# eradiate/eradiate-kernel

Measured on AMD Instinct MI355X. Metric: Msamples/s volpath 512x512x1024spp plane-parallel atmosphere, higher is better.
Workload: dtype f32; 1 GPU; C3 volpath heterogeneous 128^3 grid + HG g=0.8, 512x512x1024spp; integrator=volpath, sampler=independent seed 0, block_size=32, rfilter=box

## Files before the change

eradiate-kernel_amd/csrc/pmath.h:

```cpp
#pragma once
#include <stdint.h>
#include <math.h>
#include <string.h>

#if defined(__HIPCC__)
#  define PM_HD __host__ __device__ inline
#else
#  define PM_HD static inline
#endif

PM_HD uint32_t pm_bits(float x) { return __builtin_bit_cast(uint32_t, x); }
PM_HD float pm_from_bits(uint32_t u) { return __builtin_bit_cast(float, u); }
PM_HD uint64_t pm_bits_d(double x) { return __builtin_bit_cast(uint64_t, x); }
PM_HD double pm_from_bits_d(uint64_t u) { return __builtin_bit_cast(double, u); }

PM_HD float pm_fma(float a, float b, float c) { return __builtin_fmaf(a, b, c); }
PM_HD float pm_sqrt(float x) { return __builtin_sqrtf(x); }
PM_HD float pm_rcp(float x) {
#if defined(__HIP_DEVICE_COMPILE__) && !defined(PM_RCP_BY_DIVISION)
    const float y0 = __builtin_amdgcn_rcpf(x);
    const float e = __builtin_fmaf(-x, y0, 1.0f);
    return __builtin_amdgcn_div_fixupf(__builtin_fmaf(e, y0, y0), x, 1.0f);
#else
    return 1.0f / x;
#endif
}
PM_HD float pm_rsqrt(float x) { return pm_rcp(__builtin_sqrtf(x)); }
PM_HD float pm_abs(float x) { return pm_from_bits(pm_bits(x) & 0x7fffffffu); }

PM_HD float pm_invariant_rcp(float d) {
    const uint32_t b = pm_bits(d), e = (b >> 23) & 0xffu;
    const float rd = 1.0f / d;
    const uint32_t er = (pm_bits(rd) >> 23) & 0xffu;
    return (d > 0.f && e >= 67u && e <= 187u && er >= 67u && er <= 187u && (b & 0x7fffffu) != 0x7fffffu) ? rd : 0.f;
}
PM_HD float pm_div_by_invariant(float x, float d, float rd) {
    if (rd == 0.f || pm_bits(x) * 2u - 0x41000000u >= 0x7c000000u) return x / d;
    float q = x * rd;
    float r = pm_fma(-q, d, x);
    q = pm_fma(r, rd, q);
    r = pm_fma(-q, d, x);
    q = pm_fma(r, rd, q);
    return q;
}
PM_HD float pm_min(float a, float b) { return b < a ? b : a; }
PM_HD float pm_max(float a, float b) { return a < b ? b : a; }
PM_HD float pm_safe_sqrt(float x) { return __builtin_sqrtf(pm_max(x, 0.0f)); }
PM_HD float pm_floor(float x) { return __builtin_floorf(x); }
PM_HD float pm_ceil(float x) { return __builtin_ceilf(x); }
PM_HD float pm_inf() { return pm_from_bits(0x7f800000u); }
PM_HD float pm_nan() { return pm_from_bits(0x7fc00000u); }
PM_HD int pm_isfinite(float x) { return (pm_bits(x) & 0x7f800000u) != 0x7f800000u; }

PM_HD float pm_sign(float x) { return pm_from_bits((pm_bits(x) & 0x80000000u) | 0x3f800000u); }
PM_HD float pm_mulsign(float a, float b) { return pm_from_bits(pm_bits(a) ^ (pm_bits(b) & 0x80000000u)); }
PM_HD float pm_mulsign_neg(float a, float b) { return pm_from_bits(pm_bits(a) ^ (~pm_bits(b) & 0x80000000u)); }

PM_HD double pm_fma_d(double a, double b, double c) { return __builtin_fma(a, b, c); }

PM_HD double pm_log_core_cr(uint32_t ix) {
    int e = (int) (ix >> 23) - 126;
    float mf = pm_from_bits((ix & 0x007fffffu) | 0x3f000000u);
    if (mf < 0.707106781186547524f) { e -= 1; mf = mf + mf; }
    float tf = mf + 1.0f;
    float yf = pm_fma(pm_fma(0x1.deab9f5bac12fp-4f, tf, -0x1.71e431e019c40p-1f), tf, 0x1.7a4e362d364a6p+0f);
    yf = pm_fma(yf, pm_fma(-tf, yf, 1.0f), yf);
    double m = (double) mf, t = m + 1.0, y = (double) yf;
    y = pm_fma_d(y, pm_fma_d(-t, y, 1.0), y);
    y = pm_fma_d(y, pm_fma_d(-t, y, 1.0), y);
    double s = (m - 1.0) * y;
    double z = s * s;
    double p = 0x1.58dd5ccd0ae5bp-3;
    p = pm_fma_d(p, z, 0x1.7322766efc727p-3);
    p = pm_fma_d(p, z, 0x1.c722d2919c869p-3);
    p = pm_fma_d(p, z, 0x1.249240ad6fd9fp-2);
    p = pm_fma_d(p, z, 0x1.999999a448740p-2);
    p = pm_fma_d(p, z, 0x1.5555555552cebp-1);
    p = pm_fma_d(p, z, 0x1.0000000000001p+1);
    return pm_fma_d((double) e, 0.69314718055994530942, s * p);
}

PM_HD float pm_log_cr(float x) {
    uint32_t ix = pm_bits(x);
    if (ix >= 0x7f800000u) {
        if (ix == 0x7f800000u) return x;
        if ((ix << 1) == 0u) return -pm_inf();
        return pm_nan();
    }
    if (ix < 0x00800000u) return -pm_inf();
    return (float) pm_log_core_cr(ix);
}

PM_HD double pm_exp_d_cr(double x) {
    double fn = __builtin_floor(pm_fma_d(x, 1.44269504088896340736, 0.5));
    double r = pm_fma_d(fn, -0.693147180369123816490, x);
    r = pm_fma_d(fn, -1.90821492927058770002e-10, r);
    double p = 0x1.2727a88044faap-22;
    p = pm_fma_d(p, r, 0x1.72f98543deccbp-19);
    p = pm_fma_d(p, r, 0x1.a01b6ce393267p-16);
    p = pm_fma_d(p, r, 0x1.a0197a4e9bd9dp-13);
    p = pm_fma_d(p, r, 0x1.6c16c0c0acbd4p-10);
    p = pm_fma_d(p, r, 0x1.1111112d4977ep-7);
    p = pm_fma_d(p, r, 0x1.55555555933c2p-5);
    p = pm_fma_d(p, r, 0x1.555555554bc09p-3);
    p = pm_fma_d(p, r, 0x1.ffffffffffe17p-2);
    p = pm_fma_d(p, r, 0x1.000000000001dp+0);
    p = pm_fma_d(p, r, 1.0);
    int64_t n = (int64_t) (int) fn;
    return pm_from_bits_d(pm_bits_d(p) + ((uint64_t) n << 52));
}

PM_HD float pm_exp_cr(float x) {
    if (!(x == x)) return x;
    if (x > 88.7228317f) return pm_inf();
    if (x < -87.3365402f) return 0.0f;
    double r = pm_exp_d_cr((double) x);
    return r < 1.17549435082228750797e-38 ? 0.0f : (float) r;
}

PM_HD void pm_sincos_cr(float x, float *s_out, float *c_out) {
    double xd = (double) x;
    double fj = __builtin_floor(pm_fma_d(xd, 0.63661977236758134308, 0.5));
    double r = pm_fma_d(fj, -1.57079632673412561417, xd);
    r = pm_fma_d(fj, -6.07710050650619224932e-11, r);
    double z = r * r;
    double sp = -0x1.a950a7cb0bcc1p-26;
// ... 30 lines not shown
    float af = pm_from_bits(ax);
    float rf = pm_from_bits(0x54a232a0u - ax / 3u);
    for (int i = 0; i < 2; ++i) {
        float ar3 = af * rf * rf * rf;
        rf = rf * pm_fma(ar3, -0.333333333f, 1.33333333f);
    }
    double a = (double) af, r = (double) rf;
    for (int i = 0; i < 2; ++i) {
        double ar3 = a * r * r * r;
        r = r * pm_fma_d(ar3, -0.33333333333333333333, 1.33333333333333333333);
    }
    float y = (float) (a * r * r);
    return pm_from_bits(pm_bits(y) | sign);
}

PM_HD float pm_pow_cr(float x, float y) {
    if ((pm_bits(y) & 0x7fffffffu) < 0x00800000u) return 1.0f;
    if (!(x == x) || !(y == y)) return pm_nan();
    if (pm_bits(x) > 0x807fffffu) return pm_nan();
    if (pm_bits(x) < 0x00800000u)
        return y > 0.0f ? 0.0f : pm_inf();
    if (pm_bits(x) == 0x7f800000u) return y > 0.0f ? pm_inf() : 0.0f;
    double t = (double) y * pm_log_core_cr(pm_bits(x));
    if (t > 88.8) return pm_inf();
    if (t < -87.3365402) return 0.0f;
    float r = (float) pm_exp_d_cr(t);
    return r < 1.17549435e-38f ? 0.0f : r;
}

#define PM_LOGF_TAB_INIT {  \
    0x1.661ec79f8f3bep+0, -0x1.57bf7808caadep-2, 0x1.571ed4aaf883dp+0, -0x1.2bef0a7c06ddbp-2, \
    0x1.49539f0f010bp+0, -0x1.01eae7f513a67p-2, 0x1.3c995b0b80385p+0, -0x1.b31d8a68224e9p-3, \
    0x1.30d190c8864a5p+0, -0x1.6574f0ac07758p-3, 0x1.25e227b0b8eap+0, -0x1.1aa2bc79c81p-3, \
    0x1.1bb4a4a1a343fp+0, -0x1.a4e76ce8c0e5ep-4, 0x1.12358f08ae5bap+0, -0x1.1973c5a611cccp-4, \
    0x1.0953f419900a7p+0, -0x1.252f438e10c1ep-5, 0x1p+0, 0x0p+0, \
    0x1.e608cfd9a47acp-1, 0x1.aa5aa5df25984p-5, 0x1.ca4b31f026aap-1, 0x1.c5e53aa362eb4p-4, \
    0x1.b2036576afce6p-1, 0x1.526e57720db08p-3, 0x1.9c2d163a1aa2dp-1, 0x1.bc2860d22477p-3, \
    0x1.886e6037841edp-1, 0x1.1058bc8a07ee1p-2, 0x1.767dcf5534862p-1, 0x1.4043057b6ee09p-2 }
#define PM_LOG2F_TAB_INIT {  \
    -0x1.efec65b963019p-2, -0x1.b0b6832d4fca4p-2, -0x1.7418b0a1fb77bp-2, -0x1.39de91a6dcf7bp-2, \
    -0x1.01d9bf3f2b631p-2, -0x1.97c1d1b3b7afp-3, -0x1.2f9e393af3c9fp-3, -0x1.960cbbf788d5cp-4, \
    -0x1.a6f9db6475fcep-5, 0x0p+0, 0x1.338ca9f24f53dp-4, 0x1.476a9543891bap-3, \
    0x1.e840b4ac4e4d2p-3, 0x1.40645f0c6651cp-2, 0x1.88e9c2c1b9ff8p-2, 0x1.ce0a44eb17bccp-2 }
#define PM_EXP2F_TAB_INIT {  \
    0x3ff0000000000000ull, 0x3fefd9b0d3158574ull, 0x3fefb5586cf9890full, 0x3fef9301d0125b51ull, \
    0x3fef72b83c7d517bull, 0x3fef54873168b9aaull, 0x3fef387a6e756238ull, 0x3fef1e9df51fdee1ull, \
    0x3fef06fe0a31b715ull, 0x3feef1a7373aa9cbull, 0x3feedea64c123422ull, 0x3feece086061892dull, \
    0x3feebfdad5362a27ull, 0x3feeb42b569d4f82ull, 0x3feeab07dd485429ull, 0x3feea47eb03a5585ull, \
    0x3feea09e667f3bcdull, 0x3fee9f75e8ec5f74ull, 0x3feea11473eb0187ull, 0x3feea589994cce13ull, \
    0x3feeace5422aa0dbull, 0x3feeb737b0cdc5e5ull, 0x3feec49182a3f090ull, 0x3feed503b23e255dull, \
    0x3feee89f995ad3adull, 0x3feeff76f2fb5e47ull, 0x3fef199bdd85529cull, 0x3fef3720dcef9069ull, \
    0x3fef5818dcfba487ull, 0x3fef7c97337b9b5full, 0x3fefa4afa2a490daull, 0x3fefd0765b6e4540ull }
static const double pm_host_logf_tab[32] = PM_LOGF_TAB_INIT;
static const double pm_host_log2f_tab[16] = PM_LOG2F_TAB_INIT;
static const uint64_t pm_host_exp2f_tab[32] = PM_EXP2F_TAB_INIT;
#if defined(__HIPCC__)
static __constant__ const double pm_dev_logf_tab[32] = PM_LOGF_TAB_INIT;
static __constant__ const double pm_dev_log2f_tab[16] = PM_LOG2F_TAB_INIT;
static __constant__ const uint64_t pm_dev_exp2f_tab[32] = PM_EXP2F_TAB_INIT;
#endif
#if defined(__HIP_DEVICE_COMPILE__) && defined(PM_TABLES_IN_LDS)
__shared__ __attribute__((aligned(16))) double pm_lds_logf_tab[32];
__shared__ __attribute__((aligned(16))) uint64_t pm_lds_exp2f_tab[32];
__device__ inline void pm_tables_to_lds(uint32_t tid) {
    if (tid < 32u) { pm_lds_logf_tab[tid] = pm_dev_logf_tab[tid]; pm_lds_exp2f_tab[tid] = pm_dev_exp2f_tab[tid]; }
}
#  define PM_LOGF_TAB pm_lds_logf_tab
#  define PM_LOG2F_TAB pm_dev_log2f_tab
#  define PM_EXP2F_TAB pm_lds_exp2f_tab
#elif defined(__HIP_DEVICE_COMPILE__)
__device__ inline void pm_tables_to_lds(uint32_t) {}
#  define PM_LOGF_TAB pm_dev_logf_tab
#  define PM_LOG2F_TAB pm_dev_log2f_tab
#  define PM_EXP2F_TAB pm_dev_exp2f_tab
#else
#  if defined(__HIPCC__)
__device__ inline void pm_tables_to_lds(uint32_t) {}
#  endif
#  define PM_LOGF_TAB pm_host_logf_tab
#  define PM_LOG2F_TAB pm_host_log2f_tab
#  define PM_EXP2F_TAB pm_host_exp2f_tab
#endif

PM_HD float pm_log(float x) {
#if defined(PM_USE_LIBM) && !defined(__HIPCC__)
    return logf(x);
#endif
#if defined(PM_CORRECTLY_ROUNDED)
    return pm_log_cr(x);
#endif
    uint32_t ix = pm_bits(x);
    if (__builtin_expect(ix - 0x00800000u >= 0x7f000000u, 0)) {
        if (ix == 0x7f800000u) return x;
        if ((ix << 1) == 0u) return -pm_inf();
        if (ix < 0x00800000u) return -pm_inf();
        return pm_nan();
    }
    uint32_t tmp = ix - 0x3f330000u;
    uint32_t i = (tmp >> 19) & 15u;
    int k = (int32_t) tmp >> 23;
    double z = (double) pm_from_bits(ix - (tmp & 0xff800000u));
    double invc = PM_LOGF_TAB[2 * i], logc = PM_LOGF_TAB[2 * i + 1];
    double r = pm_fma_d(z, invc, -1.0);
    double y0 = pm_fma_d((double) k, 0x1.62e42fefa39efp-1, logc);
    double r2 = r * r;
    double y = pm_fma_d(0x1.5575b0be00b6ap-2, r, -0x1.ffffef20a4123p-2);
    y = pm_fma_d(-0x1.00ea348b88334p-2, r2, y);
    y = pm_fma_d(y, r2, y0 + r);
    return (float) y;
}

PM_HD double pm_exp2_tail(uint64_t ki, double r, double c0, double c1, double c2) {
    double s = pm_from_bits_d(PM_EXP2F_TAB[ki & 31u] + (ki << 47));
    double z = pm_fma_d(c0, r, c1);
    double r2 = r * r;
    double y = pm_fma_d(c2, r, 1.0);
    y = pm_fma_d(z, r2, y);
    return y * s;
}

PM_HD float pm_exp(float x) {
#if defined(PM_USE_LIBM) && !defined(__HIPCC__)
    return expf(x);
#endif
#if defined(PM_CORRECTLY_ROUNDED)
    return pm_exp_cr(x);
#endif
    if (__builtin_expect((pm_bits(x) & 0x7fffffffu) > 0x42aeac4fu, 0)) {
        if (!(x == x)) return x;
        if (x > 88.7228317f) return pm_inf();
        if (x < 0.0f) return 0.0f;
    }
    double xd = (double) x;
    double z = 0x1.71547652b82fep+5 * xd;
    double kd = z + 0x1.8p+52;
    uint64_t ki = pm_bits_d(kd);
    kd = kd - 0x1.8p+52;
    double r = pm_fma_d(0x1.71547652b82fep+5, xd, -kd);
    double y = pm_exp2_tail(ki, r, 0x1.c6af84b912394p-20, 0x1.ebfce50fac4f3p-13, 0x1.62e42ff0c52d6p-6);
    return y < 1.17549435082228750797e-38 ? 0.0f : (float) y;
}

PM_HD float pm_sinf_poly(double x, double x2, bool neg, int n) {
    if ((n & 1) == 0) {
        double x3 = x * x2;
        double s1 = pm_fma_d(x2, -0x1.994eb3774cf24p-13, 0x1.1107605230bc4p-7);
        double x7 = x3 * x2;
        double s = pm_fma_d(x3, -0x1.555545995a603p-3, x);
        return (float) pm_fma_d(x7, s1, s);
    }
    double sg = neg ? -1.0 : 1.0;
    double x4 = x2 * x2;
    double c2 = pm_fma_d(x2, sg * 0x1.99343027bf8c3p-16, sg * -0x1.6c087e89a359dp-10);
    double c1 = pm_fma_d(x2, sg * -0x1.ffffffd0c621cp-2, sg);
    double x6 = x4 * x2;
    double c = pm_fma_d(x4, sg * 0x1.55553e1068f19p-5, c1);
    return (float) pm_fma_d(x6, c2, c);
}

PM_HD void pm_sincos(float x, float *s_out, float *c_out) {
#if defined(PM_USE_LIBM) && !defined(__HIPCC__)
    *s_out = sinf(x); *c_out = cosf(x); return;
#endif
#if defined(PM_CORRECTLY_ROUNDED)
    pm_sincos_cr(x, s_out, c_out); return;
#endif
    uint32_t top = (pm_bits(x) >> 20) & 0x7ffu;
    double xd = (double) x;
    if (top < 0x3f4u) {
        if (top < 0x398u) { *s_out = x; *c_out = 1.0f; return; }
        double x2 = xd * xd;
        *s_out = pm_sinf_poly(xd, x2, false, 0);
        *c_out = pm_sinf_poly(xd, x2, false, 1);
        return;
    }
    if (top >= 0x42fu) { pm_sincos_cr(x, s_out, c_out); return; }
    double r = xd * 0x1.45f306dc9c883p+23;
    int n = ((int32_t) r + 0x800000) >> 24;
    xd = pm_fma_d(-(double) n, 0x1.921fb54442d18p+0, xd);
    double sg = ((n + 1) & 2) ? -1.0 : 1.0;
    double x2 = xd * xd;
    *s_out = pm_sinf_poly(xd * sg, x2, (n & 2) != 0, n);
    *c_out = pm_sinf_poly(xd * sg, x2, (n & 2) != 0, n ^ 1);
}

PM_HD float pm_cbrt(float x) {
#if defined(PM_USE_LIBM) && !defined(__HIPCC__)
    return cbrtf(x);
#endif
#if defined(PM_CORRECTLY_ROUNDED)
    return pm_cbrt_cr(x);
#endif
    uint32_t ix = pm_bits(x);
    uint32_t sign = ix & 0x80000000u;
    uint32_t ax = ix & 0x7fffffffu;
    if (ax >= 0x7f800000u) return x;
    if (ax < 0x00800000u) return pm_from_bits(sign);
    int xe = (int) (ax >> 23) - 126;
    float xm = pm_from_bits((ax & 0x007fffffu) | 0x3f000000u);
    float u = (float) (0.492659620528969547 + (0.697570460207922770 - 0.191502161678719066 * (double) xm) * (double) xm);
    float t2 = u * u * u;
    int rem = xe % 3, q = xe / 3;
    double f = rem == 0 ? 1.0 : rem == 1 ? 1.2599210498948731648 : rem == 2 ? 1.5874010519681994748
             : rem == -1 ? 1.0 / 1.2599210498948731648 : 1.0 / 1.5874010519681994748;
    float ym = (float) ((double) u * ((double) t2 + 2.0 * (double) xm) / (2.0 * (double) t2 + (double) xm) * f);
    float y = ym * pm_from_bits((uint32_t) (q + 127) << 23);
    return pm_from_bits(pm_bits(y) | sign);
}

PM_HD float pm_pow(float x, float y) {
#if defined(PM_USE_LIBM) && !defined(__HIPCC__)
    return powf(x, y);
#endif
#if defined(PM_CORRECTLY_ROUNDED)
    return pm_pow_cr(x, y);
#endif
    if ((pm_bits(y) & 0x7fffffffu) < 0x00800000u) return 1.0f;
    if (!(x == x) || !(y == y)) return pm_nan();
    if (pm_bits(x) > 0x807fffffu) return pm_nan();
    uint32_t ix = pm_bits(x);
    if (ix < 0x00800000u)
        return y > 0.0f ? 0.0f : pm_inf();
    if (ix == 0x7f800000u) return y > 0.0f ? pm_inf() : 0.0f;
// ... 25 lines not shown
```

eradiate-kernel_amd/csrc/volpath_flat.h:

```cpp
#pragma once
#include "integrator_dev.h"

namespace mtsamd {
inline namespace MTS_VARIANT_NS {

#if MTS_SPEC_N == 3
#define MTS_CX
#define MTS_CXI(id)
#define MTS_SPEC_DW 3
#else
#define MTS_CX , cx
#define MTS_CXI(id) , cx, (id)
#define MTS_SPEC_DW 4
#endif

#if MTS_SPEC_N == 3
#define MTS_FILM_STRIDE(sc) ((size_t) 5)
#else
#define MTS_FILM_STRIDE(sc) ((size_t) (sc).film_channels)
#endif
#ifndef MTS_CHAIN
#define MTS_CHAIN 1
#endif
#ifndef MTS_REPEAT_MIN_W
#define MTS_REPEAT_MIN_W 32
#endif
#define MTS_REPEAT_MIN 32

enum : uint32_t { S_TOP = 0, S_MED = 1, S_SURF = 2, S_PHASE = 3, S_BSDF = 4, S_DIRB = 5, S_NEW = 6, S_DONE = 7, S_SCATTER = 8,
                  S_ENDNEE = 9, S_ENDDIR0 = 10 };
enum : uint32_t { M_MAIN = 0, M_NEE = 1, M_DIR = 2 };
enum : uint32_t { FL_ALIVE = 1, FL_VALID_RAY = 2, FL_SPEC_CHAIN = 4, FL_NEEDS_INT = 8, FL_FROM_MEDIUM = 16 };

struct MedStep { float t, mint; F3 p; Spec sigma_t, sigma_s, combined; uint32_t info; float inv_combined ; };

DEV float div_by_invariant(float x, float d, float rd) { return pm_div_by_invariant(x, d, rd); }
DEV Spec div_by_invariant(Spec x, Spec d, float rd) {
    if (rd == 0.f) return x / d;
#if MTS_SPEC_N == 3
    return f3(div_by_invariant(x.x, d.x, rd), div_by_invariant(x.y, d.x, rd), div_by_invariant(x.z, d.x, rd));
#else
    return spec4(div_by_invariant(x.x, d.x, rd), div_by_invariant(x.y, d.x, rd), div_by_invariant(x.z, d.x, rd), div_by_invariant(x.w, d.x, rd));
#endif
}
enum : uint32_t { MI_HOMOGENEOUS = 1, MI_SPECTRAL = 2, MI_SAMPLE_EMITTERS = 4, MI_GREY = 8, MI_PHASE_SHIFT = 8 + 8 };

#if defined(MTSAMD_BLOCKSTATS)
__device__ unsigned long long g_blockstats[48];
#endif

struct GridCell { int32_t r00, r10, r01, r11, x0, x1; F3 w0, w1; };
DEV GridCell grid_cell_clamp(const float *w2l, int affine, int nx, int ny, int nz, int sx , F3 p_world) {
    F3 p = affine ? mat_point_affine(w2l, p_world) : mat_point(w2l, p_world);
    p = f3(pm_fma(p.x, (float) nx, -.5f), pm_fma(p.y, (float) ny, -.5f), pm_fma(p.z, (float) nz, -.5f));
    int ix = (int) pm_floor(p.x), iy = (int) pm_floor(p.y), iz = (int) pm_floor(p.z);
    GridCell c;
    c.w1 = p - f3((float) ix, (float) iy, (float) iz); c.w0 = f3(1.f - c.w1.x, 1.f - c.w1.y, 1.f - c.w1.z);
    c.x0 = min(max(ix, 0), nx - 1); c.x1 = min(max(ix + 1, 0), nx - 1);
    int y0 = min(max(iy, 0), ny - 1), y1 = min(max(iy + 1, 0), ny - 1), z0 = min(max(iz, 0), nz - 1), z1 = min(max(iz + 1, 0), nz - 1);
    c.r00 = (z0 * ny + y0) * sx; c.r10 = (z0 * ny + y1) * sx; c.r01 = (z1 * ny + y0) * sx; c.r11 = (z1 * ny + y1) * sx;
    return c;
}
DEV GridCell grid_cell(const DVolume &v, F3 p_world) {
    F3 p = v.affine ? mat_point_affine(v.w2l, p_world) : mat_point(v.w2l, p_world);
    const int nx = v.nx, ny = v.ny, nz = v.nz;
    p = f3(pm_fma(p.x, (float) nx, -.5f), pm_fma(p.y, (float) ny, -.5f), pm_fma(p.z, (float) nz, -.5f));
    int ix = (int) pm_floor(p.x), iy = (int) pm_floor(p.y), iz = (int) pm_floor(p.z);
    GridCell c;
    c.w1 = p - f3((float) ix, (float) iy, (float) iz); c.w0 = f3(1.f - c.w1.x, 1.f - c.w1.y, 1.f - c.w1.z);
    c.x0 = wrap_coord(v.wrap, ix, nx); c.x1 = wrap_coord(v.wrap, ix + 1, nx);
    int y0 = wrap_coord(v.wrap, iy, ny), y1 = wrap_coord(v.wrap, iy + 1, ny), z0 = wrap_coord(v.wrap, iz, nz), z1 = wrap_coord(v.wrap, iz + 1, nz);
    c.r00 = (z0 * ny + y0) * nx; c.r10 = (z0 * ny + y1) * nx; c.r01 = (z1 * ny + y0) * nx; c.r11 = (z1 * ny + y1) * nx;
    return c;
}
DEV float grid_fetch1(const MTS_GLOBAL_AS float *__restrict__ D, const GridCell &c) {
    return trilerp(D[c.r00 + c.x0], D[c.r00 + c.x1], D[c.r10 + c.x0], D[c.r10 + c.x1],
                   D[c.r01 + c.x0], D[c.r01 + c.x1], D[c.r11 + c.x0], D[c.r11 + c.x1], c.w0, c.w1);
}

typedef float mts_float4 __attribute__((ext_vector_type(4)));
typedef mts_float4 __attribute__((aligned(8))) mts_float4_a8;
DEV void grid_fetch_pair(const MTS_GLOBAL_AS float *__restrict__ P, const GridCell &c, int nx, bool columns_equal, float &sigma_t, float &albedo) {
    const int xb = min(c.x0, nx - 2);
    const bool hi0 = c.x0 != xb, hi1 = c.x1 != xb;
    mts_float4 q00 = *(const MTS_GLOBAL_AS mts_float4_a8 *) (P + 2 * (c.r00 + xb)), q01 = *(const MTS_GLOBAL_AS mts_float4_a8 *) (P + 2 * (c.r01 + xb)), q10 = q00, q11 = q01;
    if (!columns_equal) { q10 = *(const MTS_GLOBAL_AS mts_float4_a8 *) (P + 2 * (c.r10 + xb)); q11 = *(const MTS_GLOBAL_AS mts_float4_a8 *) (P + 2 * (c.r11 + xb)); }
    sigma_t = trilerp(hi0 ? q00.z : q00.x, hi1 ? q00.z : q00.x, hi0 ? q10.z : q10.x, hi1 ? q10.z : q10.x,
                      hi0 ? q01.z : q01.x, hi1 ? q01.z : q01.x, hi0 ? q11.z : q11.x, hi1 ? q11.z : q11.x, c.w0, c.w1);
    albedo = trilerp(hi0 ? q00.w : q00.y, hi1 ? q00.w : q00.y, hi0 ? q10.w : q10.y, hi1 ? q10.w : q10.y,
                     hi0 ? q01.w : q01.y, hi1 ? q01.w : q01.y, hi0 ? q11.w : q11.y, hi1 ? q11.w : q11.y, c.w0, c.w1);
}

template <bool COUNT>
DEV MedStep medium_step(const DScene &sc, const DMedium m, const DRay &ray, float sample, uint32_t channel, bool want_albedo, Counters &cnt,
                        const SpecCtx &cx = SpecCtx()) {
    MedStep mi;
#if (MTS_TRAITS & MT_MEDIA) && MTS_SPEC_N == 3
    const bool m_homogeneous = false, m_pair = true, m_grey = true, m_spectral = true;
#elif MTS_TRAITS & MT_MEDIA
    const bool m_homogeneous = false, m_pair = false, m_grey = false, m_spectral = true;
#elif MTS_TRAITS & MT_HOMOG
    const bool m_homogeneous = true, m_pair = false, m_grey = m.grey != 0, m_spectral = m.has_spectral_extinction != 0;
#else
    const bool m_homogeneous = m.is_homogeneous != 0, m_pair = m.pair_grid != nullptr, m_grey = m.grey != 0, m_spectral = m.has_spectral_extinction != 0;
#endif
    bool active = true; float mint = 0.f, maxt = pm_inf();
    if (!m_homogeneous) {
        active = bbox_ray_intersect(m.aabb, ray, mint, maxt);
        active = active && (pm_isfinite(mint) || pm_isfinite(maxt));
        if (!active) { mint = 0.f; maxt = pm_inf(); }
    }
    mint = pm_max(ray.mint, mint);
    maxt = pm_min(ray.maxt, maxt);
    Spec combined = m_homogeneous ? volume_eval(cload(sc.volumes + m.sigma_t), ray.o MTS_CXI(m.sigma_t)) * m.scale : spec_s(m.max_density);
    float mext = pick(combined, channel);
// ... 431 lines not shown
        if (MODEK == 1 && p.mode == M_MAIN) return;
        const uint32_t max_depth = (uint32_t) sc.integrator.max_depth;
        const float u = p.rng.next_1d();
        MedStep mi;
        const SpecCtx cx = ctx(p); (void) cx;
        WATERFALL_BEGIN(p.medium, mu)
            mi = medium_step<COUNT>(sc, cload(sc.media + mu), p.ray, u, p.channel, MODEK == 0 ? true : (MODEK == 1 ? false : p.mode == M_MAIN), cnt MTS_CX);
        WATERFALL_END
        if (p.si.t < mi.t) mi.t = pm_inf();
        const MediumKind mk = { mi.info };
        const bool spectral = mk.spectral(), homogeneous = mk.homogeneous(), grey = mk.grey();
        const Spec sigma_n = homogeneous ? spec_s(0.f) : mi.combined - mi.sigma_t;
        const uint32_t channel = p.channel;
        const bool is_main = MODEK == 0 ? true : (MODEK == 1 ? false : p.mode == M_MAIN), is_nee = MODEK == 0 ? false : p.mode == M_NEE;
        const float remaining_dist = is_nee ? p.ray.maxt : pm_inf();
        Spec weight = is_main ? p.thr : p.trans;
        if (spectral) {
            float t = pm_min(mi.t, p.si.t);
            if (is_nee) t = pm_min(remaining_dist, t);
            t = t - mi.mint;
            const bool surface_first = p.si.t < mi.t || mi.t > remaining_dist;
            if (grey || !homogeneous) {
                float tr = pm_exp(-t * mi.combined.x);
                float tr_pdf = surface_first ? tr : tr * mi.combined.x;
                weight = weight * (tr_pdf > 0.f ? tr * pm_rcp(tr_pdf) : 0.f);
            } else {
                Spec tr = transmittance_exp(t, mi.combined);
                Spec free_flight_pdf = surface_first ? tr : tr * mi.combined;
                float tr_pdf = pick(free_flight_pdf, channel);
                weight = weight * (tr_pdf > 0.f ? tr / tr_pdf : spec_s(0.f));
            }
        }
        float u2 = 0.f;
        if (is_main) u2 = p.rng.next_1d();
        if (is_nee) {
            if (mi.t > remaining_dist && mi.t != pm_inf()) p.wa = p.wb;
            if (mi.t > remaining_dist) mi.t = pm_inf();
        }
        const bool valid = mi.t != pm_inf();
        if (!valid) {
            if (is_main) p.thr = weight; else p.trans = weight;
            p.st = S_SURF;
            return;
        }
        const bool real_scatter = is_main && !(u2 >= (grey ? div_by_invariant(mi.sigma_t.x, mi.combined.x, mi.inv_combined)
                                                                : div_by_invariant(pick(mi.sigma_t, channel), pick(mi.combined, channel), mi.inv_combined)));
        if (!real_scatter) {
            if (grey) {
                if (is_main) { if (spectral) weight = weight * ((sigma_n.x * mi.combined.x) * pm_rcp(sigma_n.x)); }
                else { if (spectral) weight = weight * sigma_n.x; else weight = weight * div_by_invariant(sigma_n.x, mi.combined.x, mi.inv_combined); }
            } else {
                if (is_main) { if (spectral) weight = weight * (sigma_n * pick(mi.combined, channel) / pick(sigma_n, channel)); }
                else { if (spectral) weight = weight * sigma_n; else weight = weight * div_by_invariant(sigma_n, mi.combined, mi.inv_combined); }
            }
            if (is_nee) p.wa += mi.t;
            p.ray.o = mi.p; p.ray.mint = 0.f; p.si.t = p.si.t - mi.t;
            p.st = S_TOP;
            if (is_main) p.thr = weight;
            else {
                p.trans = weight;
                if (!any_nonzero(weight)) {
                    if (DEFER) p.st = is_nee ? S_ENDNEE : S_ENDDIR0;
                    else if (is_nee) end_nee(p, e); else end_direct(p, e, spec_s(0.f), 0.f);
                }
            }
            return;
        }
        p.depth += 1;
        if (!(p.depth < max_depth)) { p.thr = weight; p.flags &= ~FL_ALIVE; p.st = S_TOP; return; }
        if (grey) {
            if (spectral) weight = weight * ((mi.sigma_s.x * mi.combined.x) * pm_rcp(mi.sigma_t.x));
            else weight = weight * (mi.sigma_s.x / mi.sigma_t.x);
        } else {
            if (spectral) weight = weight * (mi.sigma_s * pick(mi.combined, channel) / pick(mi.sigma_t, channel));
            else weight = weight * (mi.sigma_s / mi.sigma_t);
        }
        p.thr = weight;
        const bool sample_emitters = (mi.info & MI_SAMPLE_EMITTERS) != 0;
        p.flags |= FL_VALID_RAY;
        p.flags = sample_emitters ? (p.flags & ~FL_SPEC_CHAIN) : (p.flags | FL_SPEC_CHAIN);
        p.ray.o = mi.p;
        p.st = sample_emitters ? S_SCATTER : S_PHASE;
    }
    template <class E> DEV void blk_scatter(PathState &p, const E &e) const {
        if (p.st != S_SCATTER) return;
        p.st = S_PHASE;
        Spec emitter_val;
        const SpecCtx cx = ctx(p); (void) cx;
        DirSample ds = sample_emitter_direction(sc, p.ray.o, p.rng.next_2d(), false, emitter_val MTS_CX);
        if (ds.pdf == 0.f) return;
        float phase_val = 0.f;
        WATERFALL_BEGIN(p.medium, mu)
            phase_val = phase_eval<true>(sc, cload(sc.media + mu).phase, -p.ray.d, p.ray.o, ds.d MTS_CX);
        WATERFALL_END
        e.cold.put_spec(C_CW, p.thr * phase_val); e.cold.put_spec(C_EMIT, emitter_val);
        e.cold.put3(C_SO, p.ray.o); e.cold.put3(C_SD, p.ray.d); e.cold.f(C_SMED) = __int_as_float(p.medium);
        p.trans = spec_s(1.f); p.wa = 0.f; p.wb = ds.dist;
        p.ray = spawn_ray(p.ray.o, ds.d); p.ray.mint = 0.f;
        queue_intersection(p);
        p.flags |= FL_FROM_MEDIUM;
        p.mode = M_NEE; p.st = S_TOP;
    }
    template <class E> DEV void blk_wsurf(PathState &p, const E &e) const {
        if (p.st != S_SURF || p.mode == M_MAIN || (p.flags & FL_NEEDS_INT)) return;
        const bool hit = hit_valid(p.si);
        const bool is_nee = p.mode == M_NEE;
        if (is_nee) p.wa += p.si.t;
        int emitter = is_nee ? -1 : sc.environment;
        Surf sf; sf.wi = -p.ray.d; sf.sh.n = f3s(0.f); sf.n = f3s(0.f);
        Spec nt = spec_s(0.f); int is_tr = 0, ext = -1, inte = -1;
        if (hit) {
            WATERFALL_BEGIN(p.si.shape, su)
                const DShape s = cload(sc.shapes + su);
                if (!is_nee) emitter = s.emitter;
                nt = s.bsdf_type == MTS_BSDF_NULL ? spec_s(1.f) : spec_s(0.f);
                is_tr = s.is_medium_transition; ext = s.exterior; inte = s.interior;
                if (emitter >= 0) complete_surface(sc, s, p.si, p.ray.d, sf);
                else if (is_tr) sf.n = hit_geo_normal(sc, s, p.si);
            WATERFALL_END
        }
        if (emitter >= 0) {
            const F3 ref_p = e.cold.get3(C_SO);
            DirSample ds;
            ds.p = p.si.p; ds.n = sf.sh.n; ds.d = p.si.p - ref_p; ds.dist = norm(ds.d); ds.d = ds.d / ds.dist;
            if (!hit) ds.d = -sf.wi;
            ds.emitter = emitter; ds.pdf = 0.f; ds.delta = false;
            const SpecCtx cx = ctx(p); (void) cx;
            end_direct(p, e, emitter_eval(sc, emitter, sf.wi.z MTS_CX), pdf_emitter_direction(sc, ref_p, ds));
            return;
        }
        if (hit) {
            p.trans = p.trans * nt;
            p.ray = spawn_ray(p.si.p, p.ray.d);
            queue_intersection(p);
            if (is_tr) p.medium = dot(p.ray.d, sf.n) > 0 ? ext : inte;
        }
        if (hit && any_nonzero(p.trans)) p.st = S_TOP;
        else if (is_nee) end_nee(p, e);
        else end_direct(p, e, spec_s(0.f), 0.f);
    }
    template <class E> DEV void blk_surf(PathState &p, const E &e) const {
        if (p.st != S_SURF || p.mode != M_MAIN || (p.flags & FL_NEEDS_INT)) return;
        const uint32_t max_depth = (uint32_t) sc.integrator.max_depth;
        const bool hit = hit_valid(p.si);
        Surf sf; sf.wi = -p.ray.d; sf.n = f3s(0.f); sf.sh.s = sf.sh.t = sf.sh.n = f3s(0.f);
        int emitter = sc.environment, bsdf_id = 0;
        if (hit) {
            WATERFALL_BEGIN(p.si.shape, su)
                const DShape s = cload(sc.shapes + su);
                emitter = s.emitter; bsdf_id = s.bsdf;
                if (s.emitter >= 0 || (s.bsdf_flags & F_Smooth) != 0) complete_surface(sc, s, p.si, p.ray.d, sf);
            WATERFALL_END
        }
        const SpecCtx cx = ctx(p); (void) cx;
        if ((p.flags & FL_SPEC_CHAIN) && emitter >= 0) p.res = p.res + p.thr * emitter_eval(sc, emitter, sf.wi.z MTS_CX);
        if (!hit) { p.flags &= ~FL_ALIVE; p.st = S_TOP; return; }
        p.st = S_BSDF;
        bool active_e = false;
        WATERFALL_BEGIN(bsdf_id, bu)
            active_e = (cload(sc.bsdfs + bu).flags & F_Smooth) != 0 && (p.depth + 1 < max_depth);
        WATERFALL_END
        if (!active_e) return;
        Spec emitter_val;
        DirSample ds = sample_emitter_direction(sc, p.si.p, p.rng.next_2d(), false, emitter_val MTS_CX);
        if (ds.pdf == 0.f) return;
        F3 wo = to_local(sf.sh, ds.d);
// ... 239 lines not shown
        if (M & G_MAXT) p.ray.maxt = f(H_MAXT);
        if (M & G_SIT) p.si.t = f(H_SIT);
        if (M & G_SIX) { p.si.p = get3(H_SIX); p.si.uv.x = f(H_SIX + 3); p.si.uv.y = f(H_SIX + 4); p.si.shape = (int) u(H_SIX + 5); p.si.prim = (int) u(H_SIX + 6); }
        if (M & G_MED) p.medium = (int) u(H_MEDIUM);
        if (M & G_THR) p.thr = get_spec(H_THR);
        if (M & G_RES) p.res = get_spec(H_RES);
        if (M & G_ETA) p.eta = f(H_ETA);
        if (M & G_TRANS) p.trans = get_spec(H_TRANS);
        if (M & G_WA) p.wa = f(H_WA);
        if (M & G_WB) p.wb = f(H_WB);
#if MTS_SPEC_N != 3
        if (M & G_WL) p.wl = get_spec(H_WL);
#endif
    }
    DEV void store(const PathState &p, int cls) const { store_m<G_ALL>(p, cls); }
    DEV void load(PathState &p) const { load_m<G_ALL>(p); }
};

struct WgArgs {
    DScene sc; const DBlock *blocks; uint32_t n_blocks, block_size, sample_count; float *film; float *cold_g; uint32_t cold_stride;
    unsigned long long *counters;
    const uint32_t *stop_flag;
    const uint32_t *tiles; uint32_t n_tiles;
};
#define MTS_TILE_PIXELS 16u

template <int WG>
DEV bool wg_env(const WgArgs &a, uint32_t wg_base, uint32_t pid, PathEnvT<ColdStoreHbm> &e) {
    const uint32_t ppb = a.block_size * a.block_size;
    e.sample_count = a.sample_count; e.film = as_global(a.film);
    e.cold.base = as_global(a.cold_g) + (size_t) (wg_base + pid) * MTS_COLD_RECORD; e.cold.stride = 1;
    __builtin_assume(((uintptr_t) e.cold.base & 127u) == 0);
    e.park = as_global(a.cold_g) + ((size_t) a.cold_stride + wg_base + pid) * MTS_COLD_RECORD;
    e.lx = e.ly = 0; e.index = 0;
    if (a.tiles != nullptr) {
        const uint32_t slot = (wg_base + pid) / MTS_TILE_PIXELS;
        if (slot >= a.n_tiles) return false;
        const uint32_t ent = as_global(a.tiles)[slot];
        if (ent == 0xFFFFFFFFu) return false;
        const MTS_GLOBAL_AS int32_t *bp = (const MTS_GLOBAL_AS int32_t *) as_global(a.blocks + (ent >> 12));
        e.blk.ox = bp[0]; e.blk.oy = bp[1]; e.blk.sx = bp[2]; e.blk.sy = bp[3]; e.blk.id = (uint32_t) bp[4]; e.blk.sample_base = (uint32_t) bp[5];
        e.blk.film_off_lo = (uint32_t) bp[6]; e.blk.film_off_hi = (uint32_t) bp[7];
        e.index = ((ent & 4095u) * MTS_TILE_PIXELS) | (pid & (MTS_TILE_PIXELS - 1u));
    } else {
        const uint32_t b = wg_base >> (uint32_t) __builtin_ctz(ppb);
        e.index = (wg_base & (ppb - 1u)) + pid;
        if (b >= a.n_blocks) return false;
        e.blk = cload(a.blocks + b);
    }
    e.film += ((size_t) e.blk.film_off_hi << 32) | e.blk.film_off_lo;
    e.lx = compact_bits(e.index); e.ly = compact_bits(e.index >> 1);
    return e.lx < (uint32_t) e.blk.sx && e.ly < (uint32_t) e.blk.sy;
}

DEV const MTS_CONST_AS void *block_uniforms(const MTS_CONST_AS void *kernarg_, uint32_t wg_base_, uint32_t &wg_base) {
    const uint64_t ka = (uint64_t) (uintptr_t) kernarg_;
    uint32_t ka_lo = (uint32_t) __builtin_amdgcn_readfirstlane((int) (uint32_t) ka), ka_hi = (uint32_t) __builtin_amdgcn_readfirstlane((int) (uint32_t) (ka >> 32));
    asm volatile("" : "+s"(ka_lo), "+s"(ka_hi));
    const MTS_CONST_AS void *kernarg = (const MTS_CONST_AS void *) (uintptr_t) ((uint64_t) ka_lo | ((uint64_t) ka_hi << 32));
    wg_base = (uint32_t) __builtin_amdgcn_readfirstlane((int) wg_base_);
    return kernarg;
}

template <bool COUNT, int WG, int C, bool WF = false, bool MOMENT = false>
#ifndef WG_BLOCK_ATTR
#define WG_BLOCK_ATTR __forceinline__
#endif
static __device__ WG_BLOCK_ATTR int wg_block(const MTS_CONST_AS void *kernarg_, uint32_t *hot_lds, uint32_t wg_base_, uint32_t pid, Counters *cnt) {
    uint32_t wg_base;
    const MTS_CONST_AS void *kernarg = block_uniforms(kernarg_, wg_base_, wg_base);
    const WgArgs a = cload_k<WgArgs>(kernarg);
    VolpathMachine<COUNT, MOMENT> vm(a.sc, *cnt);
    PathEnvT<ColdStoreHbm> e; wg_env<WG>(a, wg_base, pid, e);
    HotStore<WG> hs; hs.base = hot_lds + pid;
    typedef ClassFields<C> CF;
    PathState p;
    if (COUNT && C == B_MED) MTS_SEG_BEGIN(*cnt);
    hs.template load_m<CF::load>(p);
    if (WF && C != B_INT) p.rng.inc = wavefront_increment(a.sc.sensor, e.blk, e.lx, e.ly, __float_as_uint(e.cold.f(C_SAMPLE)));
    if (COUNT && C == B_MED) MTS_SEG(*cnt, 0);
    int cls;
#pragma nounroll
    for (int rounds = 0;; ++rounds) {
        vm.template run<CF::defer, true>(p, e, C);
        if (COUNT && C == B_MED) MTS_SEG(*cnt, 3);
        vm.template top<CF::defer>(p, e);
        if (MTS_FUSE_INT && (C == B_PHASE || C == B_SCATTER || C == B_WSURF || C == B_SURF || C == B_NEW) && a.sc.bvh_node_count == 0) {
            vm.blk_int(p, e);
            vm.template top<CF::defer>(p, e);
        }
        if (COUNT && C == B_MED) MTS_SEG(*cnt, 4);
        cls = vm.classify(p);
        if ((MTS_CHAIN & 16) && C == B_SURF) {
            if (cls != C || rounds >= 1) break;
            continue;
        }
        if ((MTS_CHAIN & 1) && C == B_WSURF) {
            if (cls != C || rounds >= 1) break;
            continue;
        }
        if (!(C == B_MED || C == B_MEDW) || cls != C || rounds >= 16) break;
        if (__popcll(__ballot(true)) < (C == B_MEDW ? MTS_REPEAT_MIN_W : MTS_REPEAT_MIN)) break;
    }
    bool chained = false;
    if ((MTS_CHAIN & 4) && C == B_MEDW && cls == B_WSURF) {
        hs.template load_add<G_ALL & ~CF::load>(p);
#pragma nounroll
        for (int r = 0; r < 2; ++r) {
            vm.blk_wsurf(p, e);
            vm.top(p, e);
            cls = vm.classify(p);
            if (cls != B_WSURF) break;
        }
        chained = true;
    }
    if ((MTS_CHAIN & 2) && (C == B_WSURF || chained) && cls == B_PHASE) {
        vm.blk_phase(p, e);
        vm.top(p, e);
        cls = vm.classify(p);
    }
    if ((MTS_CHAIN & 8) && C == B_MED && cls == B_SCATTER) {
        vm.blk_scatter(p, e);
        vm.template top<true>(p, e);
        cls = vm.classify(p);
        hs.template store_m<CF::store | ClassFields<B_SCATTER>::store>(p, cls);
    } else
    if (chained) hs.template store_m<G_ALL>(p, cls);
    else hs.template store_m<CF::store>(p, cls);
    if (COUNT && C == B_MED) MTS_SEG(*cnt, 5);
    if (CF::defer && (p.st == S_ENDNEE || p.st == S_ENDDIR0)) {
        PathState q;
        hs.template load_m<G_ALL>(q);
        if (WF) q.rng.inc = wavefront_increment(a.sc.sensor, e.blk, e.lx, e.ly, __float_as_uint(e.cold.f(C_SAMPLE)));
        vm.finish(q, e);
        vm.top(q, e);
        cls = vm.classify(q);
        hs.template store_m<G_ALL>(q, cls);
    }
    return cls;
}

template <bool COUNT_, int WG_, bool WF, bool MOMENT = false>
struct VolpathRing {
    static constexpr bool COUNT = COUNT_;
    static constexpr int WG = WG_, HOT_DWORDS = H_COUNT, PACKED = H_PACKED;
    typedef PathState State;
    typedef HotStore<WG_> Hot;
    typedef VolpathMachine<COUNT_, MOMENT> Machine;
    template <int NT> DEV static void check_shape() { static_assert(NT <= WG_, "a thread per path at most"); }
    DEV static void init_idle(State &p) {
        p.medium = -1; p.thr = p.res = p.trans = spec_s(0.f); p.eta = 1.f; p.depth = 0; p.channel = 0; p.mode = M_MAIN; p.flags = 0; p.wa = p.wb = 0.f;
#if MTS_SPEC_N != 3
        p.wl = spec_s(0.f);
#endif
    }
    template <int C> static constexpr auto block = &wg_block<COUNT_, WG_, C, WF, MOMENT>;
};

}
}
```

Measured before the change: 639.9 Msamples/s.

## Add branchless fast path for medium delta-tracking steps with rare-case fallback

Adds a specialised step_fast routine for the B_MED and B_MEDW classes in RGB media builds. It fuses medium sampling, grid lookup, transmittance, Russian roulette and state transitions into one straight-line, select-based sequence. The log, exp and invariant-division helpers gain flag variants, so the special-case checks become a single rare flag. Lanes that hit edge cases fall back to the original blk_med and top path under a wave-wide ballot. This aims to cut divergence and state-machine overhead in the hot medium loop, at the cost of duplicated logic that must stay numerically equivalent to the general path.

```diff
diff --git a/eradiate-kernel_amd/csrc/pmath.h b/eradiate-kernel_amd/csrc/pmath.h
--- a/eradiate-kernel_amd/csrc/pmath.h
+++ b/eradiate-kernel_amd/csrc/pmath.h
@@ -34,14 +34,21 @@
     const uint32_t er = (pm_bits(rd) >> 23) & 0xffu;
     return (d > 0.f && e >= 67u && e <= 187u && er >= 67u && er <= 187u && (b & 0x7fffffu) != 0x7fffffu) ? rd : 0.f;
 }
-PM_HD float pm_div_by_invariant(float x, float d, float rd) {
-    if (rd == 0.f || pm_bits(x) * 2u - 0x41000000u >= 0x7c000000u) return x / d;
+PM_HD float pm_div_by_invariant_core(float x, float d, float rd) {
     float q = x * rd;
     float r = pm_fma(-q, d, x);
     q = pm_fma(r, rd, q);
     r = pm_fma(-q, d, x);
     q = pm_fma(r, rd, q);
     return q;
+}
+PM_HD float pm_div_by_invariant(float x, float d, float rd) {
+    if (rd == 0.f || pm_bits(x) * 2u - 0x41000000u >= 0x7c000000u) return x / d;
+    return pm_div_by_invariant_core(x, d, rd);
+}
+PM_HD float pm_div_by_invariant_flag(float x, float d, float rd, bool *ok) {
+    *ok = !(pm_bits(x) * 2u - 0x41000000u >= 0x7c000000u);
+    return pm_div_by_invariant_core(x, d, rd);
 }
 PM_HD float pm_min(float a, float b) { return b < a ? b : a; }
 PM_HD float pm_max(float a, float b) { return a < b ? b : a; }
@@ -238,20 +245,7 @@
 #  define PM_EXP2F_TAB pm_host_exp2f_tab
 #endif
 
-PM_HD float pm_log(float x) {
-#if defined(PM_USE_LIBM) && !defined(__HIPCC__)
-    return logf(x);
-#endif
-#if defined(PM_CORRECTLY_ROUNDED)
-    return pm_log_cr(x);
-#endif
-    uint32_t ix = pm_bits(x);
-    if (__builtin_expect(ix - 0x00800000u >= 0x7f000000u, 0)) {
-        if (ix == 0x7f800000u) return x;
-        if ((ix << 1) == 0u) return -pm_inf();
-        if (ix < 0x00800000u) return -pm_inf();
-        return pm_nan();
-    }
+PM_HD float pm_log_core(uint32_t ix) {
     uint32_t tmp = ix - 0x3f330000u;
     uint32_t i = (tmp >> 19) & 15u;
     int k = (int32_t) tmp >> 23;
@@ -265,6 +259,31 @@
     y = pm_fma_d(y, r2, y0 + r);
     return (float) y;
 }
+PM_HD float pm_log(float x) {
+#if defined(PM_USE_LIBM) && !defined(__HIPCC__)
+    return logf(x);
+#endif
+#if defined(PM_CORRECTLY_ROUNDED)
+    return pm_log_cr(x);
+#endif
+    uint32_t ix = pm_bits(x);
+    if (__builtin_expect(ix - 0x00800000u >= 0x7f000000u, 0)) {
+        if (ix == 0x7f800000u) return x;
+        if ((ix << 1) == 0u) return -pm_inf();
+        if (ix < 0x00800000u) return -pm_inf();
+        return pm_nan();
+    }
+    return pm_log_core(ix);
+}
+PM_HD float pm_log_flag(float x, bool *ok) {
+#if (defined(PM_USE_LIBM) && !defined(__HIPCC__)) || defined(PM_CORRECTLY_ROUNDED)
+    *ok = true; return pm_log(x);
+#else
+    const uint32_t ix = pm_bits(x);
+    *ok = !(ix - 0x00800000u >= 0x7f000000u);
+    return pm_log_core(ix);
+#endif
+}
 
 PM_HD double pm_exp2_tail(uint64_t ki, double r, double c0, double c1, double c2) {
     double s = pm_from_bits_d(PM_EXP2F_TAB[ki & 31u] + (ki << 47));
@@ -275,18 +294,7 @@
     return y * s;
 }
 
-PM_HD float pm_exp(float x) {
-#if defined(PM_USE_LIBM) && !defined(__HIPCC__)
-    return expf(x);
-#endif
-#if defined(PM_CORRECTLY_ROUNDED)
-    return pm_exp_cr(x);
-#endif
-    if (__builtin_expect((pm_bits(x) & 0x7fffffffu) > 0x42aeac4fu, 0)) {
-        if (!(x == x)) return x;
-        if (x > 88.7228317f) return pm_inf();
-        if (x < 0.0f) return 0.0f;
-    }
+PM_HD float pm_exp_core(float x) {
     double xd = (double) x;
     double z = 0x1.71547652b82fep+5 * xd;
     double kd = z + 0x1.8p+52;
@@ -295,6 +303,28 @@
     double r = pm_fma_d(0x1.71547652b82fep+5, xd, -kd);
     double y = pm_exp2_tail(ki, r, 0x1.c6af84b912394p-20, 0x1.ebfce50fac4f3p-13, 0x1.62e42ff0c52d6p-6);
     return y < 1.17549435082228750797e-38 ? 0.0f : (float) y;
+}
+PM_HD float pm_exp(float x) {
+#if defined(PM_USE_LIBM) && !defined(__HIPCC__)
+    return expf(x);
+#endif
+#if defined(PM_CORRECTLY_ROUNDED)
+    return pm_exp_cr(x);
+#endif
+    if (__builtin_expect((pm_bits(x) & 0x7fffffffu) > 0x42aeac4fu, 0)) {
+        if (!(x == x)) return x;
+        if (x > 88.7228317f) return pm_inf();
+        if (x < 0.0f) return 0.0f;
+    }
+    return pm_exp_core(x);
+}
+PM_HD float pm_exp_flag(float x, bool *ok) {
+#if (defined(PM_USE_LIBM) && !defined(__HIPCC__)) || defined(PM_CORRECTLY_ROUNDED)
+    *ok = true; return pm_exp(x);
+#else
+    *ok = !((pm_bits(x) & 0x7fffffffu) > 0x42aeac4fu);
+    return pm_exp_core(x);
+#endif
 }
 
 PM_HD float pm_sinf_poly(double x, double x2, bool neg, int n) {
diff --git a/eradiate-kernel_amd/csrc/volpath_flat.h b/eradiate-kernel_amd/csrc/volpath_flat.h
--- a/eradiate-kernel_amd/csrc/volpath_flat.h
+++ b/eradiate-kernel_amd/csrc/volpath_flat.h
@@ -31,6 +31,12 @@
                   S_ENDNEE = 9, S_ENDDIR0 = 10 };
 enum : uint32_t { M_MAIN = 0, M_NEE = 1, M_DIR = 2 };
 enum : uint32_t { FL_ALIVE = 1, FL_VALID_RAY = 2, FL_SPEC_CHAIN = 4, FL_NEEDS_INT = 8, FL_FROM_MEDIUM = 16 };
+
+#if (MTS_TRAITS & MT_MEDIA) && MTS_SPEC_N == 3 && !defined(MTSAMD_BLOCKSTATS) && !defined(MTS_STEP_GENERAL)
+#define MTS_STEP_FAST 1
+#else
+#define MTS_STEP_FAST 0
+#endif
 
 struct MedStep { float t, mint; F3 p; Spec sigma_t, sigma_s, combined; uint32_t info; float inv_combined ; };
 
@@ -628,6 +634,130 @@
         p.ray.o = mi.p;
         p.st = sample_emitters ? S_SCATTER : S_PHASE;
     }
+#if MTS_STEP_FAST
+    template <int MODEK, class E> DEV int step_fast(PathState &p, const E &e) const {
+        static_assert(MODEK == 0 || MODEK == 1, "one class of the ring driver");
+        constexpr bool is_main = MODEK == 0;
+        const uint32_t max_depth = (uint32_t) sc.integrator.max_depth, rr_depth = (uint32_t) sc.integrator.rr_depth;
+        Pcg32 rng = p.rng;
+        const float u = rng.next_1d();
+        bool rare = false, valid_mi = false, sample_emitters = false;
+        float mint = 0.f, mext = 0.f, rd = 0.f, mi_t = pm_inf(), sig_t = 0.f, sig_s = 0.f;
+        F3 mi_p = f3s(0.f);
+        WATERFALL_BEGIN(p.medium, mu)
+            const DMedium m = cload(sc.media + mu);
+            if (m.inv_max_density == 0.f) rare = true;
+            else {
+                float bmint, bmaxt;
+                bool active = bbox_ray_intersect(m.aabb, p.ray, bmint, bmaxt);
+                active = active && (pm_isfinite(bmint) || pm_isfinite(bmaxt));
+                bmint = active ? bmint : 0.f; bmaxt = active ? bmaxt : pm_inf();
+                mint = pm_max(p.ray.mint, bmint);
+                const float maxt = pm_min(p.ray.maxt, bmaxt);
+                mext = m.max_density; rd = m.inv_max_density;
+                bool ok_log, ok_div;
+                const float sampled_t = mint + pm_div_by_invariant_flag(-pm_log_flag(1.f - u, &ok_log), mext, rd, &ok_div);
+                rare = !(ok_log && ok_div);
+                valid_mi = active && (sampled_t <= maxt);
+                mi_t = valid_mi ? sampled_t : pm_inf();
+                mi_p = ray_at(p.ray, sampled_t);
+                const bool look = valid_mi && !rare;
+                const F3 at = f3(look ? mi_p.x : p.ray.o.x, look ? mi_p.y : p.ray.o.y, look ? mi_p.z : p.ray.o.z);
+                const int sx = m.pair_nx < 2 ? 2 : m.pair_nx;
+                const GridCell c = grid_cell_clamp(m.pair_w2l, m.pair_affine & 1, m.pair_nx, m.pair_ny, m.pair_nz, sx, at);
+                float st_raw, al_raw;
+                grid_fetch_pair(as_global(m.pair_grid), c, sx, (m.pair_affine & 2) != 0, st_raw, al_raw);
+                sig_t = m.scale * st_raw;
+                if (is_main) sig_s = sig_t * al_raw;
+                sample_emitters = m.sample_emitters != 0;
+            }
+        WATERFALL_END
+        const float si_t = p.si.t;
+        mi_t = si_t < mi_t ? pm_inf() : mi_t;
+        const bool is_nee = !is_main && p.mode == M_NEE;
+        const float remaining_dist = is_nee ? p.ray.maxt : pm_inf();
+        Spec weight = is_main ? p.thr : p.trans;
+        float t = pm_min(mi_t, si_t);
+        if (!is_main) t = is_nee ? pm_min(remaining_dist, t) : t;
+        t = t - mint;
+        const bool surface_first = si_t < mi_t || mi_t > remaining_dist;
+        bool ok_exp;
+        const float tr = pm_exp_flag(-t * mext, &ok_exp);
+        rare = rare || !ok_exp;
+        const float tr_pdf = surface_first ? tr : tr * mext;
+        weight = weight * (tr_pdf > 0.f ? tr * pm_rcp(tr_pdf) : 0.f);
+        float u2 = 0.f;
+        if (is_main) u2 = rng.next_1d();
+        float wa = p.wa;
+        if (!is_main) {
+            wa = (mi_t > remaining_dist && mi_t != pm_inf()) ? p.wb : wa;
+            mi_t = mi_t > remaining_dist ? pm_inf() : mi_t;
+        }
+        const bool valid = mi_t != pm_inf();
+        const float sigma_n = mext - sig_t;
+        int cls;
+        if (is_main) {
+            bool ok_div2;
+            const float ratio = pm_div_by_invariant_flag(sig_t, mext, rd, &ok_div2);
+            const bool real = valid && !(u2 >= ratio);
+            const uint32_t depth1 = p.depth + 1u;
+            rare = rare || (valid && !ok_div2) || (real && !(depth1 < max_depth));
+            const float factor = real ? (sig_s * mext) * pm_rcp(sig_t) : (sigma_n * mext) * pm_rcp(sigma_n);
+            const Spec stepped = weight * factor;
+            Spec thr = f3(valid ? stepped.x : weight.x, valid ? stepped.y : weight.y, valid ? stepped.z : weight.z);
+            bool alive = (p.flags & FL_ALIVE) && any_nonzero(thr);
+            const float q = pm_min(hmax(thr) * (p.eta * p.eta), .95f);
+            const bool perform_rr = p.depth > rr_depth;
+            Pcg32 rng_head = rng;
+            alive = alive && (rng_head.next_1d() < q || !perform_rr);
+            const Spec thr_rr = thr * pm_rcp(q);
+            const bool null_c = valid && !real, rr_c = null_c && perform_rr;
+            const bool ends = !alive || p.depth >= max_depth;
+            thr = f3(rr_c ? thr_rr.x : thr.x, rr_c ? thr_rr.y : thr.y, rr_c ? thr_rr.z : thr.z);
+            const uint32_t fl = p.flags | FL_VALID_RAY;
+            const uint32_t st_real = sample_emitters ? S_SCATTER : S_PHASE, st_null = ends ? S_NEW : S_MED;
+            const int cls_real = sample_emitters ? B_SCATTER : B_PHASE, cls_null = ends ? B_NEW : B_MED;
+            cls = valid ? (real ? cls_real : cls_null) : B_SURF;
+            if (!rare) {
+                if (COUNT) { cnt.n_lookup += valid_mi ? 1u : 0u; cnt.n_iter += (null_c && !ends) ? 1u : 0u; }
+                p.thr = thr;
+                p.rng.state = null_c ? rng_head.state : rng.state;
+                p.ray.o = f3(valid ? mi_p.x : p.ray.o.x, valid ? mi_p.y : p.ray.o.y, valid ? mi_p.z : p.ray.o.z);
+                p.ray.mint = null_c ? 0.f : p.ray.mint;
+                p.si.t = null_c ? si_t - mi_t : si_t;
+                p.depth = real ? depth1 : p.depth;
+                p.flags = real ? (sample_emitters ? (fl & ~FL_SPEC_CHAIN) : (fl | FL_SPEC_CHAIN)) : p.flags;
+                p.st = valid ? (real ? st_real : st_null) : S_SURF;
+            }
+        } else {
+            const Spec stepped = weight * sigma_n;
+            rare = rare || (valid && !any_nonzero(stepped));
+            const float wa_step = is_nee ? wa + mi_t : wa;
+            const float left = p.wb * (1.f - MTS_SHADOW_EPSILON) - wa_step;
+            const bool ends = is_nee && !(left > 0.f);
+            cls = valid ? (ends ? B_NEW  : B_MEDW) : B_WSURF;
+            if (!rare) {
+                if (COUNT) { cnt.n_lookup += valid_mi ? 1u : 0u; cnt.n_nee_step += (valid && !ends) ? 1u : 0u; }
+                p.trans = f3(valid ? stepped.x : weight.x, valid ? stepped.y : weight.y, valid ? stepped.z : weight.z);
+                p.rng.state = rng.state;
+                p.wa = valid ? wa_step : wa;
+                p.ray.o = f3(valid ? mi_p.x : p.ray.o.x, valid ? mi_p.y : p.ray.o.y, valid ? mi_p.z : p.ray.o.z);
+                p.ray.mint = valid ? 0.f : p.ray.mint;
+                p.ray.maxt = (valid && is_nee) ? left : p.ray.maxt;
+                p.si.t = valid ? si_t - mi_t : si_t;
+                p.st = valid ? (ends ? S_ENDNEE : S_MED) : S_SURF;
+            }
+        }
+        if (__builtin_expect(__ballot(rare) != 0ull, 0)) {
+            if (rare) {
+                blk_med<true, MODEK>(p, e);
+                top<true>(p, e);
+                cls = Base::classify(p);
+            }
+        }
+        return cls;
+    }
+#endif
     template <class E> DEV void blk_scatter(PathState &p, const E &e) const {
         if (p.st != S_SCATTER) return;
         p.st = S_PHASE;
@@ -1033,15 +1163,21 @@
     int cls;
 #pragma nounroll
     for (int rounds = 0;; ++rounds) {
-        vm.template run<CF::defer, true>(p, e, C);
-        if (COUNT && C == B_MED) MTS_SEG(*cnt, 3);
-        vm.template top<CF::defer>(p, e);
-        if (MTS_FUSE_INT && (C == B_PHASE || C == B_SCATTER || C == B_WSURF || C == B_SURF || C == B_NEW) && a.sc.bvh_node_count == 0) {
-            vm.blk_int(p, e);
+#if MTS_STEP_FAST
+        if constexpr (C == B_MED || C == B_MEDW) cls = vm.template step_fast<C == B_MED ? 0 : 1>(p, e);
+        else
+#endif
+        {
+            vm.template run<CF::defer, true>(p, e, C);
+            if (COUNT && C == B_MED) MTS_SEG(*cnt, 3);
             vm.template top<CF::defer>(p, e);
-        }
-        if (COUNT && C == B_MED) MTS_SEG(*cnt, 4);
-        cls = vm.classify(p);
+            if (MTS_FUSE_INT && (C == B_PHASE || C == B_SCATTER || C == B_WSURF || C == B_SURF || C == B_NEW) && a.sc.bvh_node_count == 0) {
+                vm.blk_int(p, e);
+                vm.template top<CF::defer>(p, e);
+            }
+            if (COUNT && C == B_MED) MTS_SEG(*cnt, 4);
+            cls = vm.classify(p);
+        }
         if ((MTS_CHAIN & 16) && C == B_SURF) {
             if (cls != C || rounds >= 1) break;
             continue;
```

New measurement: 665.0 Msamples/s (median of 6 runs). 3.9% higher.
